# sdroh1027/DiffusionVID

Measured on AMD Instinct MI355X. Metric: frames/sec (1000x600) DiffusionVID-R101 x1, higher is better.
Workload: dtype f16

## Files before the change

### diffusionvid_amd/_lib.py

```python
import ctypes as C
import os

_HERE = os.path.dirname(os.path.abspath(__file__))
LIB_PATH = os.environ.get("DVID_LIB") or os.path.join(_HERE, "libdvid_hip.so")

c_void_p, c_int, c_float, c_int64 = C.c_void_p, C.c_int, C.c_float, C.c_int64
c_float_p = C.POINTER(C.c_float)


class DvidConfig(C.Structure):
    _fields_ = [
        ("hidden_dim", c_int), ("nheads", c_int), ("dim_feedforward", c_int), ("dim_dynamic", c_int),
        ("num_classes", c_int), ("num_cls", c_int), ("num_reg", c_int), ("num_heads", c_int),
        ("num_heads_cond", c_int), ("pooler_resolution", c_int), ("sampling_ratio", c_int),
        ("res_blocks", c_int * 4), ("pixel_mean", c_float * 3), ("pixel_std", c_float * 3),
        ("backbone_type", c_int), ("swin_embed_dim", c_int), ("swin_depths", c_int * 4), ("swin_heads", c_int * 4),
        ("swin_window", c_int),
    ]


SIGNATURES = {
    "dvid_last_error": (C.c_char_p, []),
    "dvid_version": (c_int, []),
    "dvid_model_create": (c_int, [C.POINTER(DvidConfig), C.POINTER(c_void_p)]),
# ... 40 lines not shown
    "dvid_noise_to_boxes": (c_int, [c_void_p, c_void_p, c_int, c_float, c_float, c_float, c_void_p]),
    "dvid_noise_to_boxes_sizes": (c_int, [c_void_p, c_void_p, c_int, c_int, c_float, c_void_p, c_void_p]),
    "dvid_ddim_renew_step_sizes": (c_int, [c_void_p] * 6 + [c_int] * 3 + [c_void_p] + [c_float] * 7 + [c_void_p]),
    "dvid_postproc_topk_nms_sizes": (c_int, [c_void_p, c_void_p, c_int, c_int, c_int, c_int, c_void_p, c_float, c_int,
                                             c_void_p, c_void_p, c_void_p, c_void_p, c_void_p, c_void_p]),
    "dvid_nms_frames_tiled_sizes": (c_int, [c_void_p] * 3 + [c_int, c_int, c_void_p, c_float, c_int, c_int] + [c_void_p] * 6),
    "dvid_ddim_renew_step": (c_int, [c_void_p] * 6 + [c_int] * 3 + [c_float] * 9 + [c_void_p]),
    "dvid_postproc_topk_nms": (c_int, [c_void_p, c_void_p, c_int, c_int, c_int, c_int, c_float, c_float, c_float, c_int,
                                       c_void_p, c_void_p, c_void_p, c_void_p, c_void_p, c_void_p]),
    "dvid_postproc_scratch_bytes": (c_int64, [c_int, c_int, c_int]),
    "dvid_topk_candidates_stream": (c_int, [c_void_p, c_void_p, c_int, c_int, c_int, c_int, c_void_p, c_void_p, c_void_p, c_void_p]),
    "dvid_nms_frames_tiled": (c_int, [c_void_p] * 3 + [c_int, c_int, c_float, c_float, c_float, c_int, c_int] + [c_void_p] * 6),
    "dvid_nms_tiled_scratch_bytes": (c_int64, [c_int, c_int]),
    "dvid_seq_nms_video": (c_int, [c_void_p] * 4 + [c_int] * 3 + [c_void_p] * 4 + [c_int64, c_void_p]),
    "dvid_seq_nms_scratch_bytes": (c_int64, [c_void_p, c_void_p, c_int, c_int]),
    "dvid_vid_eval_match": (c_int, [c_void_p, c_void_p, c_int, c_int] + [c_void_p] * 4 + [c_int, c_int] + [c_void_p] * 3 + [c_int, c_float, c_int] +
                            [c_void_p] * 7),
    "dvid_coco_eval_match": (c_int, [c_void_p, c_void_p, c_int, c_int] + [c_void_p] * 8 + [c_int] + [c_void_p] * 5),
    "dvid_lvis_eval_match": (c_int, [c_void_p, c_void_p, c_int, c_int] + [c_void_p] * 14 + [c_int] + [c_void_p] * 5),
    "dvid_eval_accumulate": (c_int, [c_void_p] * 6 + [c_int] * 5 + [c_void_p, c_int, c_void_p, c_int] + [c_void_p] * 3 + [c_int64, c_void_p]),
    "dvid_eval_accumulate_scratch_bytes": (c_int64, [c_int, c_int, c_int]),
    "dvid_cdist":(c_int, [c_void_p, c_int, c_int, c_void_p, c_void_p]),
    "dvid_fps_greedy": (c_int, [c_void_p, c_int, c_int, c_int, c_void_p, c_void_p]),
    "dvid_gather_rows": (c_int, [c_void_p, c_void_p, c_void_p, c_int, c_int, c_void_p]),
    "dvid_cdist_groups": (c_int, [c_void_p, c_int, c_int, c_int, c_void_p, c_void_p]),
    "dvid_fps_greedy_groups": (c_int, [c_void_p, c_int, c_int, c_int, c_int, c_void_p, c_void_p]),
    "dvid_gather_rows_groups": (c_int, [c_void_p, c_void_p, c_void_p, c_int, c_int, c_int, c_int, c_void_p]),
    "dvid_update_memory_groups": (c_int, [c_void_p, c_int, c_int, c_int, c_int, c_void_p, c_void_p, c_void_p, c_void_p]),
    "dvid_conv2d_nhwc_f16": (c_int, [c_void_p, c_void_p, c_void_p, c_void_p, c_void_p] + [c_int] * 13 + [c_void_p]),
    "dvid_bottleneck64_tail_f16": (c_int, [c_void_p] * 10 + [c_int] + [c_void_p] * 2 + [c_int] * 3 + [c_void_p]),
    "dvid_bottleneck128_tail_f16": (c_int, [c_void_p] * 10 + [c_int] * 3 + [c_void_p]),
    "dvid_mha_f16": (c_int, [c_void_p] * 5 + [c_int] * 7 + [c_int64] * 3 + [c_void_p]),
    "dvid_dynconv": (c_int, [c_void_p] * 7 + [c_int, c_void_p]),
    "dvid_add_layernorm": (c_int, [c_void_p] * 5 + [c_int, c_int, c_int, c_void_p]),
    "dvid_swin_pack_relbias": (c_int, [c_void_p, c_int, c_void_p]),
    "dvid_swin_window_attn_f16": (c_int, [c_void_p] * 4 + [c_int] * 6 + [c_void_p]),
    "dvid_swin_pack_relbias_ws": (c_int, [c_void_p, c_int, c_int, c_void_p]),
    "dvid_swin_window_attn_f16_ws": (c_int, [c_void_p] * 4 + [c_int] * 7 + [c_void_p]),
    "dvid_patch_merge_ln": (c_int, [c_void_p] * 5 + [c_int] * 4 + [c_void_p]),
    "dvid_nhwc_from_nchw": (c_int, [c_void_p, c_void_p, c_int, c_int, c_int, c_int, c_void_p]),
    "dvid_nchw_from_nhwc": (c_int, [c_void_p, c_void_p, c_int, c_int, c_int, c_int, c_void_p]),
    "dvid_f32_to_f16": (c_int, [c_void_p, c_void_p, c_int64, c_void_p]),
    "dvid_resize_u8_to_f32": (c_int, [c_void_p, c_int, c_int, c_void_p, c_void_p, c_int, c_int, c_int, c_int, c_void_p, c_void_p, c_int,
                                      c_void_p, c_void_p, c_int, c_void_p]),
    "dvid_resize_views_u8": (c_int, [c_void_p, c_int, c_void_p, c_void_p, c_void_p, c_int64, c_void_p, c_int64, c_void_p, c_int64, c_void_p, c_int, c_int,
                                     c_int, c_void_p]),
    "dvid_bbox_aug_merge": (c_int, [c_void_p] * 5 + [c_int] * 3 + [c_void_p] * 5),
    "dvid_overlay_detections": (c_int, [c_void_p] * 3 + [c_int, c_void_p, c_void_p, c_int, c_void_p, c_void_p, c_int, c_void_p, c_int, c_int,
                                        c_float, c_int, c_int, c_void_p, c_int64, c_void_p]),
    "dvid_overlay_scratch_bytes": (c_int64, [c_int, c_int]),
    "dvid_overlay_tile": (c_int, [C.POINTER(c_int), C.POINTER(c_int)]),
    "dvid_jpeg_parse": (c_int, [c_void_p, c_int64, c_void_p, c_void_p, c_int]),
    "dvid_jpeg_entropy_decode": (c_int, [c_void_p, c_int64, c_void_p, c_int64, c_void_p, c_void_p, c_int]),
    "dvid_jpeg_reconstruct_u8": (c_int, [c_void_p, c_int64, c_void_p, c_int64, c_void_p, c_void_p, c_int, c_void_p, c_int64, c_void_p, c_int64,
                                         c_void_p]),
    "dvid_igemm_num_configs": (c_int, []),
    "dvid_igemm_set_config": (c_int, [c_int]),
    "dvid_igemm_set_tuning": (c_int, [c_int]),
    "dvid_igemm_tuning_passes": (C.c_longlong, []),
    "dvid_igemm_set_conv3x3": (c_int, [c_int]),
    "dvid_igemm_set_wstat": (c_int, [c_int]),
    "dvid_igemm_set_bottleneck_fusion": (c_int, [c_int]),
    "dvid_set_stem_pool": (c_int, [c_int]),
    "dvid_set_option": (c_int, [C.c_char_p, c_int]),
    "dvid_get_option": (c_int, [C.c_char_p, C.POINTER(c_int)]),
    "dvid_reset_options": (c_int, []),
# ... 57 lines not shown
```

### diffusionvid_amd/csrc/dynconv.hip

```cpp
#include "common.h"
#include "f32_split.h"
#include "igemm_epilogue.h"
#include "kernels.h"
#include "options.h"
#include "roi_taps.h"

namespace {

constexpr int NP = 49;
constexpr int D = 256;
constexpr int DD = 64;
constexpr int A_PITCH = D + 8;
constexpr int H_PITCH = DD + 8;

__device__ __forceinline__ float groups4_sum(float v) {
    v += __shfl_xor(v, 16, 64);
    v += __shfl_xor(v, 32, 64);
    return v;
}

template <bool FUSED_ROI>
__global__ __launch_bounds__(256, 3) void dynconv_kernel(const half_t* __restrict__ roi, const half_t* __restrict__ params,
                                                       const float* __restrict__ g1, const float* __restrict__ b1,
                                                       const float* __restrict__ g2, const float* __restrict__ b2,
                                                       half_t* __restrict__ out, RoiLevels lv, const float* __restrict__ boxes,
                                                       int boxes_per_img, int nbox) {
    extern __shared__ __attribute__((aligned(16))) char smem[];
    half_t* As = reinterpret_cast<half_t*>(smem);
    half_t* Hs = As + 64 * A_PITCH;
    float* red = reinterpret_cast<float*>(Hs + 64 * H_PITCH);

    const int box = FUSED_ROI ? igemm_xcd_remap((int)blockIdx.x, nbox) : (int)blockIdx.x;
    const int tid = threadIdx.x, lane = tid & 63, wave = tid >> 6;
    const int l15 = lane & 15, l4 = lane >> 4;
    const half_t* p1t = params + (long)box * (2 * D * DD);
    const half_t* p2t = p1t + D * DD;
    const half8 zero8 = {0, 0, 0, 0, 0, 0, 0, 0};
    half8 bf[8];
    half8 b2f[4][2];

    if (FUSED_ROI) {
#pragma unroll
        for (int ks = 0; ks < 8; ++ks)
            bf[ks] = *reinterpret_cast<const half8*>(p1t + (wave * 16 + l15) * D + ks * 32 + l4 * 8);
#pragma unroll
        for (int nt = 0; nt < 4; ++nt)
#pragma unroll
            for (int ks = 0; ks < 2; ++ks)
                b2f[nt][ks] = *reinterpret_cast<const half8*>(p2t + (wave * 64 + nt * 16 + l15) * DD + ks * 32 + l4 * 8);
        float macc[8];
        roi_taps::gather_box(lv, boxes, boxes_per_img, box, tid >> 5, tid & 31, macc,
                             [&](int p, half8 o) { *reinterpret_cast<half8*>(As + p * A_PITCH + (tid & 31) * 8) = o; });
        for (int i = tid; i < (64 - NP) * 32; i += 256) *reinterpret_cast<half8*>(As + (NP + (i >> 5)) * A_PITCH + (i & 31) * 8) = zero8;
    } else {
        const half_t* roi_b = roi + (long)box * NP * D;
        for (int i = tid; i < 64 * 32; i += 256) {
            const int r = i >> 5, cv = i & 31;
            const half8 v = *reinterpret_cast<const half8*>(roi_b + (long)(r < NP ? r : 0) * D + cv * 8);
            *reinterpret_cast<half8*>(As + r * A_PITCH + cv * 8) = (r < NP) ? v : zero8;
        }
#pragma unroll
        for (int ks = 0; ks < 8; ++ks)
            bf[ks] = *reinterpret_cast<const half8*>(p1t + (wave * 16 + l15) * D + ks * 32 + l4 * 8);
    }
    __syncthreads();

    float4v acc1[4];
#pragma unroll
    for (int mt = 0; mt < 4; ++mt) acc1[mt] = (float4v){0.f, 0.f, 0.f, 0.f};
#pragma unroll
    for (int ks = 0; ks < 8; ++ks) {
#pragma unroll
        for (int mt = 0; mt < 4; ++mt) {
            const half8 af = *reinterpret_cast<const half8*>(As + (mt * 16 + l15) * A_PITCH + ks * 32 + l4 * 8);
            acc1[mt] = __builtin_amdgcn_mfma_f32_16x16x32_f16(bf[ks], af, acc1[mt], 0, 0, 0);
        }
    }
    if (!FUSED_ROI) {
#pragma unroll
        for (int nt = 0; nt < 4; ++nt)
#pragma unroll
            for (int ks = 0; ks < 2; ++ks)
                b2f[nt][ks] = *reinterpret_cast<const half8*>(p2t + (wave * 64 + nt * 16 + l15) * DD + ks * 32 + l4 * 8);
    }
// ... 90 lines not shown
    for (int nt = 0; nt < 4; ++nt) {
        const int col = wave * 64 + nt * 16 + l4 * 4;
        const float4v gg = *reinterpret_cast<const float4v*>(g2 + col), bb = *reinterpret_cast<const float4v*>(b2 + col);
#pragma unroll
        for (int mt = 0; mt < 4; ++mt) {
            half4 y;
#pragma unroll
            for (int r = 0; r < 4; ++r) y[r] = (half_t)fmaxf((acc2[mt][nt][r] - mean[mt]) * rstd[mt] * gg[r] + bb[r], 0.f);
            *reinterpret_cast<half4*>(As + (mt * 16 + l15) * A_PITCH + col) = y;
        }
    }
    __syncthreads();
    half_t* out_b = out + (long)box * NP * D;
    for (int i = tid; i < NP * 32; i += 256) {
        const int r = i >> 5, cv = i & 31;
        *reinterpret_cast<half8*>(out_b + (long)r * D + cv * 8) = *reinterpret_cast<const half8*>(As + r * A_PITCH + cv * 8);
    }
}

constexpr int kSmem = 64 * A_PITCH * 2 + 64 * H_PITCH * 2 + 64 * 4 * 4;

}

int dvid_dynconv_launch(const half_t* roi, const half_t* params, const float* g1, const float* b1, const float* g2,
                        const float* b2, half_t* out, int rows, hipStream_t s) {
    if (rows == 0) return DVID_OK;
    hipLaunchKernelGGL(dynconv_kernel<false>, dim3(rows), dim3(256), kSmem, s, roi, params, g1, b1, g2, b2, out, RoiLevels{}, nullptr, 1, rows);
    LAUNCH_CHECK();
    return DVID_OK;
}

int dvid_dynconv_roi_launch(const RoiLevels& lv, int channels, const float* boxes, int n_img, int boxes_per_img, const half_t* params,
                            const float* g1, const float* b1, const float* g2, const float* b2, half_t* out, hipStream_t s) {
    if (channels != 256) return DVID_ERR_UNSUPPORTED;
    const int rows = n_img * boxes_per_img;
    if (rows == 0) return DVID_OK;
    hipLaunchKernelGGL(dynconv_kernel<true>, dim3(rows), dim3(256), kSmem, s, nullptr, params, g1, b1, g2, b2, out, lv, boxes, boxes_per_img, rows);
    LAUNCH_CHECK();
    return DVID_OK;
}

namespace {

constexpr int DC_P1 = 68, DC_P2 = 260;
__global__ __launch_bounds__(256) __attribute__((amdgpu_waves_per_eu(2, 2))) void f32_dynconv_kernel(const float* __restrict__ roi, const float* __restrict__ params,
                                                           const float* __restrict__ g1, const float* __restrict__ b1,
                                                           const float* __restrict__ g2, const float* __restrict__ b2, float* __restrict__ out,
                                                           int nbox) {
#pragma clang fp contract(off)
    __shared__ float F1[64 * DC_P1];
    __shared__ float F2[49 * DC_P2];
    const int box = igemm_xcd_remap((int)blockIdx.x, nbox);
    const int tid = threadIdx.x, lane = tid & 63, wave = tid >> 6;
    const int fr = lane & 31, fk = (lane >> 5) * 4;
    const float* x = roi + (long)box * 49 * 256;
    const float* p1 = params + (long)box * 32768;
    const float* p2 = p1 + 64 * 256;

    float4v w2[2][8];
#pragma unroll
    for (int nb = 0; nb < 2; ++nb)
#pragma unroll
        for (int j = 0; j < 8; ++j) w2[nb][j] = *reinterpret_cast<const float4v*>(p2 + (long)((wave * 2 + nb) * 32 + fr) * 64 + j * 8 + fk);

    {
        const int mb = wave >> 1, nb = wave & 1;
        const int prow = mb * 32 + fr;
// ... 281 lines not shown
```

### diffusionvid_amd/csrc/model.hip

```cpp
#include <stdarg.h>

#include "runtime.h"

DvidOptions g_opt;

thread_local char g_err[512] = "";
void set_err(const char* fmt, ...) {
    va_list ap;
    va_start(ap, fmt);
    vsnprintf(g_err, sizeof(g_err), fmt, ap);
    va_end(ap);
}

int conv_run(const ConvW& w, const half_t* in, int n, int h, int wd, void* out, hipStream_t s, const ConvOpts& o) {
    IgemmParams p;
    memset(&p, 0, sizeof(p));
    p.in = in;
    p.w = w.w;
    p.bias = w.bias;
    p.res = o.res;
    p.out = out;
    p.H = h;
    p.W = wd;
    p.Cin = w.cin;
// ... 45 lines not shown
    p.wscale = w.wscale32;
    p.res = o.res;
    p.out = out;
    p.H = h;
    p.W = wd;
    p.Cin = w.cin32;
    p.KH = w.kh;
    p.KW = w.kw;
    p.stride = w.stride;
    p.pad = w.pad;
    p.Ho = (h + 2 * w.pad - w.kh) / w.stride + 1;
    p.Wo = (wd + 2 * w.pad - w.kw) / w.stride + 1;
    p.Cout = w.cout;
    p.M = n * p.Ho * p.Wo;
    p.K = w.kh * w.kw * w.cin32;
    p.Kpad = w.kpad32;
    p.ldc = o.ldc ? o.ldc : w.cout;
    p.relu = o.relu;
    p.res_mode = o.res_mode;
    if (o.ho_out) *o.ho_out = p.Ho;
    if (o.wo_out) *o.wo_out = p.Wo;
    const double alg_k = (double)w.kh * w.kw * (w.cin_real ? w.cin_real : w.cin32);
    const double in_px = (double)p.M * (w.kh * w.kw > 1 ? w.stride * w.stride : 1);
    const double bytes = 4.0 * (in_px * p.Cin + (double)p.Cout * p.Kpad + (double)p.M * p.Cout * (o.res_mode == 1 ? 2.0 : o.res_mode == 2 ? 1.25 : 1.0));
    return prof_other("igemm_f32", p.M, p.Cout, p.Kpad, 2.0 * p.M * (double)p.Cout * alg_k, bytes, s, [&] { return dvid_f32_igemm_launch(p, s); },
                      true);
}
int linear_run32(const ConvW& w, const float* in, int rows, float* out, int relu, hipStream_t s, int ldc) {
    return conv_run32(w, in, rows, 1, 1, out, s, {.relu = relu, .ldc = ldc});
}

extern "C" {
const char* dvid_last_error(void) { return g_err; }
int dvid_version(void) { return 11; }

int dvid_model_create(const dvid_config* cfg, dvid_model** out) {
    g_err[0] = 0;
    if (!cfg || !out) FAIL(DVID_ERR_ARG, "null argument");
    if (cfg->hidden_dim != 256 || cfg->nheads != 8 || cfg->dim_dynamic != 64 || cfg->pooler_resolution != 7 ||
        cfg->sampling_ratio != 2)
        FAIL(DVID_ERR_UNSUPPORTED,
             "kernels are specialised for HIDDEN_DIM 256, NHEADS 8, DIM_DYNAMIC 64, POOLER_RESOLUTION 7, SAMPLING_RATIO 2");
    if (cfg->dim_feedforward % 64) FAIL(DVID_ERR_UNSUPPORTED, "DIM_FEEDFORWARD must be a multiple of 64");
    if (cfg->num_classes < 1 || cfg->num_classes > DVID_MAX_CLASSES)
        FAIL(DVID_ERR_UNSUPPORTED, "NUM_CLASSES %d: 1 <= NUM_CLASSES <= DVID_MAX_CLASSES = %d", cfg->num_classes, DVID_MAX_CLASSES);
    int dev_count = 0;
    if (hipGetDeviceCount(&dev_count) != hipSuccess || dev_count == 0) FAIL(DVID_ERR_HIP, "no HIP device available");
    dvid_model* m = new dvid_model();
    m->cfg = *cfg;
    if (const char* e = getenv("DVID_CHAINS")) m->nchain = atoi(e) < 1 ? 1 : (atoi(e) > 4 ? 4 : atoi(e));
    *out = m;
    return DVID_OK;
}

int dvid_model_destroy(dvid_model* m) {
    if (!m) return DVID_OK;
    for (void* p : m->owned) (void)hipFree(p);
    delete m;
    return DVID_OK;
}

int dvid_model_set_precision(dvid_model* m, int precision) {
    g_err[0] = 0;
    if (!m || (precision != 0 && precision != 1)) FAIL(DVID_ERR_ARG, "precision must be 0 (float16) or 1 (float32)");
    if (m->finalized) FAIL(DVID_ERR_STATE, "dvid_model_set_precision must precede dvid_model_finalize (the weights are packed for one precision)");
    m->precision = precision;
    return DVID_OK;
// ... 163 lines not shown
```

### diffusionvid_amd/csrc/ops_abi.hip

```cpp
#include "runtime.h"

extern "C" {
int dvid_roialign_v2_multilevel(const void* p3, const void* p4, const void* p5, int n_frames, int height, int width, int channels,
                                const float* boxes, int boxes_per_frame, void* roi_out, float* mean_out, void* stream) {
    const void* levels[3] = {p3, p4, p5};
    return dvid_roialign_v2_levels(levels, 3, n_frames, height, width, channels, boxes, boxes_per_frame, roi_out, mean_out, stream);
}

int dvid_roialign_v2_levels(const void* const* levels, int n_levels, int n_frames, int height, int width, int channels, const float* boxes,
                            int boxes_per_frame, void* roi_out, float* mean_out, void* stream) {
    g_err[0] = 0;
    if (!pyramid_ok(levels, n_levels)) FAIL(DVID_ERR_ARG, "the pyramid is 3 maps (p3..p5) or 4 (p2..p5), none of them null (got n_levels %d)", n_levels);
    if (height % 32 || width % 32) FAIL(DVID_ERR_ARG, "height/width must be multiples of 32");
    TRY(dvid_roialign_launch(roi_levels<half_t>(levels, n_levels, height, width, 0, channels), channels, boxes, n_frames, boxes_per_frame,
                             reinterpret_cast<half_t*>(roi_out), mean_out, reinterpret_cast<hipStream_t>(stream)));
    return DVID_OK;
}

int dvid_roialign_v2_multilevel_f32(const float* p3, const float* p4, const float* p5, int n_frames, int height, int width, int channels,
                                    const float* boxes, int boxes_per_frame, float* roi_out, float* mean_out, void* stream) {
    const float* levels[3] = {p3, p4, p5};
    return dvid_roialign_v2_levels_f32(levels, 3, n_frames, height, width, channels, boxes, boxes_per_frame, roi_out, mean_out, stream);
}

// ... 483 lines not shown
    const int rc = bneck_tail(reinterpret_cast<const half_t*>(t1), reinterpret_cast<const half_t*>(w2), b2, reinterpret_cast<const half_t*>(w3),
                              b3, reinterpret_cast<const half_t*>(residual), reinterpret_cast<const half_t*>(w_shortcut), b_shortcut,
                              reinterpret_cast<const half_t*>(w1_next), b1_next, next_channels, reinterpret_cast<half_t*>(out),
                              reinterpret_cast<half_t*>(t1_next), n, h, wd, reinterpret_cast<hipStream_t>(stream));
    if (rc != DVID_OK) FAIL(rc, "bottleneck tail: bad argument (n %d, %d x %d, next conv1 with %d channels)", n, h, wd, next_channels);
    return DVID_OK;
}

int dvid_bottleneck128_tail_f16(const void* t1, const void* w2, const float* b2, const void* w3, const float* b3, const void* residual,
                                const void* w1_next, const float* b1_next, void* out, void* t1_next, int n, int h, int wd, void* stream) {
    g_err[0] = 0;
    const int rc = bneck128_tail(reinterpret_cast<const half_t*>(t1), reinterpret_cast<const half_t*>(w2), b2, reinterpret_cast<const half_t*>(w3),
                                 b3, reinterpret_cast<const half_t*>(residual), reinterpret_cast<const half_t*>(w1_next), b1_next,
                                 reinterpret_cast<half_t*>(out), reinterpret_cast<half_t*>(t1_next), n, h, wd,
                                 reinterpret_cast<hipStream_t>(stream));
    if (rc != DVID_OK) FAIL(rc, "bottleneck tail (128): bad argument (n %d, %d x %d)", n, h, wd);
    return DVID_OK;
}

int dvid_mha_f16(const void* q, const void* k, const void* v, void* out, void* vt_scratch, int batch, int lq, int lk, int nheads,
                 int q_ld, int kv_ld, int out_ld, int64_t q_bs, int64_t kv_bs, int64_t out_bs, void* stream) {
    g_err[0] = 0;
    TRY(dvid_mha_mfma_launch(reinterpret_cast<const half_t*>(q), reinterpret_cast<const half_t*>(k), reinterpret_cast<const half_t*>(v),
                             reinterpret_cast<half_t*>(out), reinterpret_cast<half_t*>(vt_scratch), batch, lq, lk, nheads, q_ld, kv_ld,
                             out_ld, q_bs, kv_bs, out_bs, reinterpret_cast<hipStream_t>(stream)));
    return DVID_OK;
}

int dvid_dynconv(const void* roi, const void* params, const float* g1, const float* b1, const float* g2, const float* b2, void* out,
                 int rows, void* stream) {
    g_err[0] = 0;
    TRY(dvid_dynconv_launch(reinterpret_cast<const half_t*>(roi), reinterpret_cast<const half_t*>(params), g1, b1, g2, b2,
                            reinterpret_cast<half_t*>(out), rows, reinterpret_cast<hipStream_t>(stream)));
    return DVID_OK;
}

int dvid_add_layernorm(const float* x, const float* r, const float* g, const float* b, float* y, int rows, int d, int relu,
                       void* stream) {
    g_err[0] = 0;
    TRY(dvid_add_layernorm_launch(x, r, g, b, y, nullptr, rows, d, relu, reinterpret_cast<hipStream_t>(stream)));
    return DVID_OK;
}

int dvid_swin_window_attn_f16(const void* qkv, const void* qkv_bias16, const float* relbias, void* out, int batch, int H, int W, int C,
                              int nheads, int shift, void* stream) {
    g_err[0] = 0;
    if (!qkv || !qkv_bias16 || !relbias || !out) FAIL(DVID_ERR_ARG, "swin window attention: null pointer");
    if (batch <= 0 || H <= 0 || W <= 0 || nheads <= 0 || shift < 0 || shift >= 7)
        FAIL(DVID_ERR_ARG, "swin window attention: bad sizes (batch %d, %d x %d tokens, %d heads, shift %d)", batch, H, W, nheads, shift);
    const int rc = dvid_swin_window_attn_launch(reinterpret_cast<const half_t*>(qkv), reinterpret_cast<const half_t*>(qkv_bias16), relbias,
                                                reinterpret_cast<half_t*>(out), batch, H, W, C, nheads, shift, reinterpret_cast<hipStream_t>(stream));
    if (rc != DVID_OK) FAIL(rc, "swin window attention: C %d with %d heads on %d x %d x %d tokens is not supported", C, nheads, batch, H, W);
    return DVID_OK;
}

int dvid_swin_window_attn_f16_ws(const void* qkv, const void* qkv_bias16, const float* relbias, void* out, int batch, int H, int W, int C,
                                 int nheads, int shift, int window, void* stream) {
    if (window == 7) return dvid_swin_window_attn_f16(qkv, qkv_bias16, relbias, out, batch, H, W, C, nheads, shift, stream);
    g_err[0] = 0;
    if (window != 12) FAIL(DVID_ERR_UNSUPPORTED, "swin window attention: window size %d (7 and 12 are built)", window);
    if (!qkv || !qkv_bias16 || !relbias || !out) FAIL(DVID_ERR_ARG, "swin window attention: null pointer");
    if (batch <= 0 || H <= 0 || W <= 0 || nheads <= 0 || shift < 0 || shift >= window)
        FAIL(DVID_ERR_ARG, "swin window attention: bad sizes (batch %d, %d x %d tokens, %d heads, shift %d, window %d)", batch, H, W, nheads, shift, window);
    const int rc = dvid_swin_window12_attn_launch(reinterpret_cast<const half_t*>(qkv), reinterpret_cast<const half_t*>(qkv_bias16), relbias,
                                                  reinterpret_cast<half_t*>(out), batch, H, W, C, nheads, shift, reinterpret_cast<hipStream_t>(stream));
    if (rc != DVID_OK) FAIL(rc, "swin window attention (window 12): C %d with %d heads on %d x %d x %d tokens is not supported", C, nheads, batch, H, W);
// ... 173 lines not shown
```

### diffusionvid_amd/csrc/roi_taps.h

```cpp
#pragma once

#include "common.h"
#include "kernels.h"

namespace roi_taps {

constexpr int P = 7;
constexpr int G = 2;
constexpr int CV = 32;

typedef unsigned int uint4v __attribute__((ext_vector_type(4)));
__device__ __forceinline__ float mix_fma_lo(unsigned int h2, float w, float acc) {
    float d;
    asm("v_fma_mix_f32 %0, %1, %2, %3 op_sel_hi:[1,0,0]" : "=v"(d) : "v"(h2), "v"(w), "v"(acc));
    return d;
}
__device__ __forceinline__ float mix_fma_hi(unsigned int h2, float w, float acc) {
    float d;
    asm("v_fma_mix_f32 %0, %1, %2, %3 op_sel:[1,0,0] op_sel_hi:[1,0,0]" : "=v"(d) : "v"(h2), "v"(w), "v"(acc));
    return d;
}
__device__ __forceinline__ void tap_fma8(float (&acc)[8], half8 v, float w) {
    const uint4v u = __builtin_bit_cast(uint4v, v);
#pragma unroll
    for (int q = 0; q < 4; ++q) {
        acc[2 * q] = mix_fma_lo(u[q], w, acc[2 * q]);
        acc[2 * q + 1] = mix_fma_hi(u[q], w, acc[2 * q + 1]);
    }
}

struct Tap {
    int lo, hi;
    float wl, wh;
    bool ok;
};

__device__ __forceinline__ Tap axis_tap(float y, int limit) {
    Tap t;
    t.ok = !(y < -1.0f || y > (float)limit);
    if (y <= 0.f) y = 0.f;
    int lo = (int)y;
    int hi;
    if (lo >= limit - 1) {
        hi = lo = limit - 1;
        y = (float)lo;
    } else {
        hi = lo + 1;
    }
    const float l = y - (float)lo;
    t.lo = lo;
    t.hi = hi;
    t.wl = 1.f - l;
    t.wh = l;
    return t;
}

__device__ __forceinline__ int box_level(float bx1, float by1, float bx2, float by2, int min_level, bool& valid) {
    const float area = (bx2 - bx1) * (by2 - by1);
    valid = area >= 0.f;
    float lvf = floorf(4.f + log2f(sqrtf(area) / 224.f + 1e-8f));
    lvf = fminf(fmaxf(lvf, (float)min_level), 5.f);
    return valid ? (int)lvf - min_level : 0;
}

template <typename Sink>
__device__ __forceinline__ void gather_box(const RoiLevels& lv, const float* __restrict__ boxes, int boxes_per_img, int box, int grp, int ln,
                                           float (&macc)[8], Sink&& sink) {
    const int img = box / boxes_per_img;
    const float bx1 = boxes[box * 4 + 0], by1 = boxes[box * 4 + 1], bx2 = boxes[box * 4 + 2], by2 = boxes[box * 4 + 3];
    bool valid_box;
    const int level = box_level(bx1, by1, bx2, by2, lv.min_level, valid_box);

    const half_t* feat = lv.feat[level];
    const int H = lv.h[level], W = lv.w[level];
    const float sc = lv.scale[level];
    feat += (long)img * H * W * (CV * 8);

    const float x1 = bx1 * sc - 0.5f, y1 = by1 * sc - 0.5f;
    const float x2 = bx2 * sc - 0.5f, y2 = by2 * sc - 0.5f;
    const float bin_w = (x2 - x1) / P, bin_h = (y2 - y1) / P;

#pragma unroll
    for (int e = 0; e < 8; ++e) macc[e] = 0.f;

    for (int p = grp; p < P * P; p += 8) {
        const int ph = p / P, pw = p - ph * P;
        float acc[8];
#pragma unroll
        for (int e = 0; e < 8; ++e) acc[e] = 0.f;
        if (valid_box) {
#pragma unroll
            for (int iy = 0; iy < G; ++iy) {
                const float y = y1 + ph * bin_h + (iy + 0.5f) * bin_h / G;
                const Tap ty = axis_tap(y, H);
#pragma unroll
                for (int ix = 0; ix < G; ++ix) {
                    const float x = x1 + pw * bin_w + (ix + 0.5f) * bin_w / G;
                    const Tap tx = axis_tap(x, W);
                    if (!(ty.ok && tx.ok)) continue;
                    const half8 v1 = *reinterpret_cast<const half8*>(feat + ((long)ty.lo * W + tx.lo) * (CV * 8) + ln * 8);
                    const half8 v2 = *reinterpret_cast<const half8*>(feat + ((long)ty.lo * W + tx.hi) * (CV * 8) + ln * 8);
                    const half8 v3 = *reinterpret_cast<const half8*>(feat + ((long)ty.hi * W + tx.lo) * (CV * 8) + ln * 8);
                    const half8 v4 = *reinterpret_cast<const half8*>(feat + ((long)ty.hi * W + tx.hi) * (CV * 8) + ln * 8);
                    const float w1 = ty.wl * tx.wl, w2 = ty.wl * tx.wh, w3 = ty.wh * tx.wl, w4 = ty.wh * tx.wh;
                    tap_fma8(acc, v1, w1);
                    tap_fma8(acc, v2, w2);
                    tap_fma8(acc, v3, w3);
                    tap_fma8(acc, v4, w4);
                }
            }
        }
        half8 o;
#pragma unroll
        for (int e = 0; e < 8; ++e) {
            acc[e] *= 1.f / (G * G);
            macc[e] += acc[e];
            o[e] = (half_t)acc[e];
        }
        sink(p, o);
    }
}

}
```

### diffusionvid_amd/csrc/roialign.hip

```cpp
#include <stdlib.h>

#include "common.h"
#include "igemm_epilogue.h"
#include "kernels.h"
#include "roi_taps.h"

namespace {

using namespace roi_taps;

__global__ __launch_bounds__(256) void roialign_kernel(RoiLevels lv, const float* __restrict__ boxes, int boxes_per_img,
                                                        half_t* __restrict__ roi_out, float* __restrict__ mean_out, int nbox,
                                                        int xcd_major) {
    __shared__ float red[8][256];
    const int box = xcd_major ? igemm_xcd_remap((int)blockIdx.x, nbox) : (int)blockIdx.x;
    const int tid = threadIdx.x;
    const int grp = tid >> 5, ln = tid & 31;
    float macc[8];
    gather_box(lv, boxes, boxes_per_img, box, grp, ln, macc,
               [&](int p, half8 o) { *reinterpret_cast<half8*>(roi_out + ((long)box * (P * P) + p) * (CV * 8) + ln * 8) = o; });
    if (mean_out) {
#pragma unroll
        for (int e = 0; e < 8; ++e) red[grp][ln * 8 + e] = macc[e];
        __syncthreads();
        float s = 0.f;
#pragma unroll
        for (int g = 0; g < 8; ++g) s += red[g][tid];
        mean_out[(long)box * 256 + tid] = s / (P * P);
    }
}

__global__ __launch_bounds__(256) void f32_roialign_kernel(RoiLevels32 lv, const float* __restrict__ boxes, int boxes_per_img,
                                                            float* __restrict__ roi_out, float* __restrict__ mean_out, int nbox) {
#pragma clang fp contract(off)
    __shared__ float red[8][256];
    const int box = igemm_xcd_remap((int)blockIdx.x, nbox);
    const int img = box / boxes_per_img;
    const int tid = threadIdx.x;
    const int grp = tid >> 5, ln = tid & 31;
    const float bx1 = boxes[box * 4 + 0], by1 = boxes[box * 4 + 1], bx2 = boxes[box * 4 + 2], by2 = boxes[box * 4 + 3];
    bool valid_box;
    const int level = box_level(bx1, by1, bx2, by2, lv.min_level, valid_box);
    const int H = lv.h[level], W = lv.w[level];
    const float sc = lv.scale[level];
    const float* feat = lv.feat[level] + (long)img * H * W * 256;
    const float x1 = bx1 * sc - 0.5f, y1 = by1 * sc - 0.5f;
    const float x2 = bx2 * sc - 0.5f, y2 = by2 * sc - 0.5f;
    const float bin_w = (x2 - x1) / P, bin_h = (y2 - y1) / P;
    float macc[8];
#pragma unroll
    for (int e = 0; e < 8; ++e) macc[e] = 0.f;
    for (int pb = grp; pb < P * P; pb += 8) {
// ... 20 lines not shown
#pragma unroll
                        for (int e = 0; e < 4; ++e) {
                            acc[e] += w4[q] * a[e];
                            acc[4 + e] += w4[q] * b[e];
                        }
                    }
                }
            }
        }
#pragma unroll
        for (int e = 0; e < 8; ++e) {
            acc[e] *= 1.f / (G * G);
            macc[e] += acc[e];
        }
        float* o = roi_out + ((long)box * (P * P) + pb) * 256 + ln * 8;
        *reinterpret_cast<float4v*>(o) = (float4v){acc[0], acc[1], acc[2], acc[3]};
        *reinterpret_cast<float4v*>(o + 4) = (float4v){acc[4], acc[5], acc[6], acc[7]};
    }
    if (mean_out) {
#pragma unroll
        for (int e = 0; e < 8; ++e) red[grp][ln * 8 + e] = macc[e];
        __syncthreads();
        float s = 0.f;
#pragma unroll
        for (int g = 0; g < 8; ++g) s += red[g][tid];
        mean_out[(long)box * 256 + tid] = s / (P * P);
    }
}

}

int dvid_roialign_launch(const RoiLevels& lv, int channels, const float* boxes, int n_img, int boxes_per_img, half_t* roi_out,
                         float* mean_out, hipStream_t s) {
    if (channels != 256) return DVID_ERR_UNSUPPORTED;
    const int nbox = n_img * boxes_per_img;
    if (nbox == 0) return DVID_OK;
    hipLaunchKernelGGL(roialign_kernel, dim3(nbox), dim3(256), 0, s, lv, boxes, boxes_per_img, roi_out, mean_out, nbox, 1);
    LAUNCH_CHECK();
    return DVID_OK;
}

int dvid_f32_roialign_launch(const RoiLevels32& lv, int channels, const float* boxes, int n_img, int boxes_per_img, float* roi_out,
                             float* mean_out, hipStream_t s) {
    if (channels != 256) return DVID_ERR_UNSUPPORTED;
    const int nbox = n_img * boxes_per_img;
    if (nbox == 0) return DVID_OK;
    hipLaunchKernelGGL(f32_roialign_kernel, dim3(nbox), dim3(256), 0, s, lv, boxes, boxes_per_img, roi_out, mean_out, nbox);
    LAUNCH_CHECK();
    return DVID_OK;
}
```

### diffusionvid_amd/ops.py

```python
import ctypes as C

import torch

from . import _lib
from ._lib import call, ptr, stream_ptr


def _cuda(t, dtype=None):
    if not t.is_cuda:
        raise _lib.DvidError("libdvid_hip ops need tensors on the GPU (no CPU fallback)")
    if dtype is not None and t.dtype != dtype:
        raise TypeError(f"expected {dtype}, got {t.dtype}")
    return t.contiguous()


def nhwc_from_nchw(x):
    x = _cuda(x, torch.float32)
    n, c, h, w = x.shape
    out = torch.empty((n, h, w, c), dtype=torch.float16, device=x.device)
    call("dvid_nhwc_from_nchw", ptr(x), ptr(out), n, h, w, c, stream_ptr())
    return out


def nchw_from_nhwc(x):
# ... 147 lines not shown
    feats = [_cuda(f, torch.float16) for f in feats_nhwc]
    levels, nl = _pyramid(feats, height, width, "roialign")
    boxes = _cuda(boxes, torch.float32)
    n, M = boxes.shape[:2]
    c = feats[0].shape[-1]
    roi = torch.empty((n * M, 49, c), dtype=torch.float16, device=boxes.device)
    mean = torch.empty((n * M, c), dtype=torch.float32, device=boxes.device) if want_mean else None
    call("dvid_roialign_v2_levels", levels, nl, n, height, width, c, ptr(boxes), M, ptr(roi), ptr(mean), stream_ptr())
    return (roi, mean) if want_mean else roi


def mha_f16(q, k, v, nheads):
    def h(t):
        t = _cuda(t)
        if t.dtype == torch.float16:
            return t
        o = torch.empty(t.shape, dtype=torch.float16, device=t.device)
        call("dvid_f32_to_f16", ptr(t), ptr(o), t.numel(), stream_ptr())
        return o
    q, k, v = h(q), h(k), h(v)
    B, lq, d = q.shape
    lk = k.shape[1]
    out = torch.empty_like(q)
    vt = torch.empty((B * nheads * 32 * ((lk + 31) // 32 * 32 + 32),), dtype=torch.float16, device=q.device)
    call("dvid_mha_f16", ptr(q), ptr(k), ptr(v), ptr(out), ptr(vt), B, lq, lk, nheads, d, d, d, lq * d, lk * d, lq * d,
         stream_ptr())
    return out


def dynconv(roi16, params16, g1, b1, g2, b2):
    roi16, params16 = _cuda(roi16, torch.float16), _cuda(params16, torch.float16)
    out = torch.empty_like(roi16)
    call("dvid_dynconv", ptr(roi16), ptr(params16), ptr(g1), ptr(b1), ptr(g2), ptr(b2), ptr(out), roi16.shape[0], stream_ptr())
    return out


def add_layernorm(x, r, g, b, relu=False):
    x = _cuda(x, torch.float32)
    y = torch.empty_like(x)
    call("dvid_add_layernorm", ptr(x), ptr(r), ptr(g), ptr(b), ptr(y), x.shape[0], x.shape[1], int(relu), stream_ptr())
    return y


def _swin_relbias_pitch(window):
    return (window * window + 31) // 32 * 32


def swin_pack_relbias(table, window=7):
    table = table.detach().cpu().contiguous()
    if table.dtype != torch.float32 or table.dim() != 2 or table.shape[0] != (2 * window - 1) ** 2:
        raise TypeError(f"expected a float32 [{(2 * window - 1) ** 2}, heads] table, got {table.dtype} {tuple(table.shape)}")
    out = torch.empty((table.shape[1], window * window, _swin_relbias_pitch(window)), dtype=torch.float32)
    if window == 7:
        call("dvid_swin_pack_relbias", ptr(table), table.shape[1], ptr(out))
    else:
        call("dvid_swin_pack_relbias_ws", ptr(table), table.shape[1], window, ptr(out))
    return out


def _swin_window_attn(name, dtype, qkv, qkv_bias, relbias, B, H, W, nheads, shift, out, window):
    qkv, qkv_bias, relbias = _cuda(qkv, dtype), _cuda(qkv_bias, dtype), _cuda(relbias, torch.float32)
    C = qkv.shape[1] // 3
    assert tuple(qkv.shape) == (B * H * W, 3 * C) and qkv_bias.numel() == 3 * C
    assert tuple(relbias.shape) == (nheads, window * window, _swin_relbias_pitch(window))
    if out is None:
        out = torch.empty((B * H * W, C), dtype=dtype, device=qkv.device)
# ... 829 lines not shown
```

### include/dvid_hip.h

```cpp
#ifndef DVID_HIP_H
#define DVID_HIP_H

#include <stdint.h>

#ifdef __cplusplus
extern "C" {
#endif

#define DVID_OK 0
#define DVID_ERR_ARG 1
#define DVID_ERR_HIP 2
#define DVID_ERR_UNSUPPORTED 3
#define DVID_ERR_STATE 4

#define DVID_MAX_CLASSES 1280

typedef struct dvid_model dvid_model;

typedef struct dvid_config {
    int hidden_dim;
    int nheads;
    int dim_feedforward;
    int dim_dynamic;
    int num_classes;
// ... 136 lines not shown
int dvid_lvis_eval_match(const float* dets, const int* counts, int n_images, int cap, const double* gt_boxes, const double* gt_areas,
                         const unsigned char* gt_ignore, const int* gt_labels, const int* gt_starts, const int* gt_starts_host,
                         const int* neg_starts, const int* neg_labels, const int* neg_starts_host, const int* nex_starts, const int* nex_labels,
                         const int* nex_starts_host, const double* iou_thrs, const double* area_ranges, int num_classes, signed char* match,
                         signed char* ignore, int* rank, int* npig, void* stream);
#define DVID_EVAL_ACCUMULATE_RECALLS 101
#define DVID_EVAL_ACCUMULATE_MAX_LIMITS 3
#define DVID_EVAL_ACCUMULATE_MAX_SCRATCH_BYTES (1ll << 30)
int dvid_eval_accumulate(const float* dets, const int* counts, const int* rank, const signed char* match, const signed char* ignore,
                         const int* npig, int n_images, int cap, int num_classes, int n_areas, int n_thresholds, const int* max_dets,
                         int max_dets_count, const double* rec_thrs, int n_rec_thrs, double* precision, double* recall, void* scratch,
                         long long scratch_bytes, void* stream);
long long dvid_eval_accumulate_scratch_bytes(int n_images, int cap, int max_dets_count);
int dvid_cdist(const float* x, int n, int d, float* dist, void* stream);
int dvid_fps_greedy(const float* dist, int n, int m, int bs_emul, int* idx, void* stream);
int dvid_gather_rows(const float* x, const int* idx, float* y, int m, int d, void* stream);
#define DVID_UPDATE_MEMORY_MAX_SCRATCH_BYTES (1ll << 30)
int dvid_cdist_groups(const float* x, int groups, int n, int d, float* dist, void* stream);
int dvid_fps_greedy_groups(const float* dist, int groups, int n, int m, int bs_emul, int* idx, void* stream);
int dvid_gather_rows_groups(const float* x, const int* idx, float* y, int groups, int n, int m, int d, void* stream);
int dvid_update_memory_groups(const float* merged, int groups, int n, int d, int m, float* dist_scratch, int* idx, float* out, void* stream);
int dvid_conv2d_nhwc_f16(const void* in, const void* w, const float* bias, const void* residual, void* out, int n, int h,
                         int wd, int cin, int cout, int kh, int kw, int stride, int pad, int kpad, int relu, int out_f32,
                         int residual_mode, void* stream);
int dvid_bottleneck64_tail_f16(const void* t1, const void* w2, const float* b2, const void* w3, const float* b3, const void* residual,
                               const void* w_shortcut, const float* b_shortcut, const void* w1_next, const float* b1_next, int next_channels,
                               void* out, void* t1_next, int n, int h, int wd, void* stream);
int dvid_bottleneck128_tail_f16(const void* t1, const void* w2, const float* b2, const void* w3, const float* b3, const void* residual,
                                const void* w1_next, const float* b1_next, void* out, void* t1_next, int n, int h, int wd, void* stream);
int dvid_mha_f16(const void* q, const void* k, const void* v, void* out, void* vt_scratch, int batch, int lq, int lk, int nheads,
                 int q_ld, int kv_ld, int out_ld, int64_t q_bs, int64_t kv_bs, int64_t out_bs, void* stream);
int dvid_dynconv(const void* roi, const void* params, const float* g1, const float* b1, const float* g2, const float* b2,
                 void* out, int rows, void* stream);
int dvid_add_layernorm(const float* x, const float* r, const float* g, const float* b, float* y, int rows, int d, int relu,
                       void* stream);
int dvid_swin_pack_relbias(const float* table, int nheads, float* out);
int dvid_swin_window_attn_f16(const void* qkv, const void* qkv_bias16, const float* relbias, void* out, int batch, int H, int W, int C,
                              int nheads, int shift, void* stream);
int dvid_swin_pack_relbias_ws(const float* table, int nheads, int window, float* out);
int dvid_swin_window_attn_f16_ws(const void* qkv, const void* qkv_bias16, const float* relbias, void* out, int batch, int H, int W, int C,
                                 int nheads, int shift, int window, void* stream);
int dvid_patch_merge_ln(const float* x, const float* g, const float* b, void* y16, float* y32, int B, int H, int W, int C, void* stream);
int dvid_nhwc_from_nchw(const float* in, void* out_f16, int n, int h, int w, int c, void* stream);
int dvid_nchw_from_nhwc(const void* in_f16, float* out, int n, int h, int w, int c, void* stream);
int dvid_f32_to_f16(const float* x, void* y, int64_t n, void* stream);

int dvid_resize_u8_to_f32(const void* src_hwc, int h, int w, void* tmp, float* out_chw, int oh, int ow, int ph, int pw,
                          const int* xbounds, const int* xk, int xksize, const int* ybounds, const int* yk, int yksize, void* stream);

int dvid_resize_views_u8(const void* const* srcs, int n, const long long* plan, const long long* plan_host, const int* bounds,
                         int64_t n_bound_rows, const int* weights, int64_t n_weights, void* tmp, int64_t tmp_bytes, float* out, int ph, int pw,
                         int flip, void* stream);
#define DVID_BBOX_AUG_MAX_VIEWS 64
int dvid_bbox_aug_merge(const float* boxes, const float* scores, const int* labels, const int* counts, const float* table, int n, int views,
                        int cap, float* cand_boxes, float* cand_scores, int* cand_labels, int* live, void* stream);

#define DVID_OVERLAY_MAX_DRAWN 256
#define DVID_OVERLAY_NAME_MAX 24
int dvid_overlay_detections(void* const* frames, const int* sizes, const int* sizes_host, int n, const float* dets, const int* counts, int cap,
                            const float* ratios, const unsigned char* names, int num_classes, const unsigned char* atlas, int gh, int gw,
                            float threshold, int thickness, int text_scale, void* scratch, int64_t scratch_bytes, void* stream);
int64_t dvid_overlay_scratch_bytes(int n, int cap);
int dvid_overlay_tile(int* tile_w, int* tile_h);

typedef struct dvid_jpeg_info {
    int32_t width, height, ncomp;
// ... 41 lines not shown
```

Before: 2378.

## Batch RoIAlign bilinear loads across samples and expose fused RoI dynconv entry point

Templates gather_box on a sample count. The standalone RoIAlign kernel now issues the loads for all four bilinear samples before accumulating, and uses 32-bit unsigned offsets, which is guarded by a new check on map size. The fused dynconv path keeps one sample at a time to limit register pressure. The change also pins down FMA contraction so results are deterministic, adds a public ABI and Python wrapper for the fused RoIAlign+DynamicConv kernel, and bumps the library version. Batching the loads costs more registers in exchange for more loads in flight.

```diff
diff --git a/diffusionvid_amd/_lib.py b/diffusionvid_amd/_lib.py
--- a/diffusionvid_amd/_lib.py
+++ b/diffusionvid_amd/_lib.py
@@ -96,6 +96,7 @@
     "dvid_bottleneck128_tail_f16": (c_int, [c_void_p] * 10 + [c_int] * 3 + [c_void_p]),
     "dvid_mha_f16": (c_int, [c_void_p] * 5 + [c_int] * 7 + [c_int64] * 3 + [c_void_p]),
     "dvid_dynconv": (c_int, [c_void_p] * 7 + [c_int, c_void_p]),
+    "dvid_dynconv_roi": (c_int, [c_void_p, c_int, c_int, c_int, c_int, c_void_p, c_int] + [c_void_p] * 7),
     "dvid_add_layernorm": (c_int, [c_void_p] * 5 + [c_int, c_int, c_int, c_void_p]),
     "dvid_swin_pack_relbias": (c_int, [c_void_p, c_int, c_void_p]),
     "dvid_swin_window_attn_f16": (c_int, [c_void_p] * 4 + [c_int] * 6 + [c_void_p]),
diff --git a/diffusionvid_amd/csrc/dynconv.hip b/diffusionvid_amd/csrc/dynconv.hip
--- a/diffusionvid_amd/csrc/dynconv.hip
+++ b/diffusionvid_amd/csrc/dynconv.hip
@@ -49,7 +49,7 @@
             for (int ks = 0; ks < 2; ++ks)
                 b2f[nt][ks] = *reinterpret_cast<const half8*>(p2t + (wave * 64 + nt * 16 + l15) * DD + ks * 32 + l4 * 8);
         float macc[8];
-        roi_taps::gather_box(lv, boxes, boxes_per_img, box, tid >> 5, tid & 31, macc,
+        roi_taps::gather_box<1>(lv, boxes, boxes_per_img, box, tid >> 5, tid & 31, macc,
                              [&](int p, half8 o) { *reinterpret_cast<half8*>(As + p * A_PITCH + (tid & 31) * 8) = o; });
         for (int i = tid; i < (64 - NP) * 32; i += 256) *reinterpret_cast<half8*>(As + (NP + (i >> 5)) * A_PITCH + (i & 31) * 8) = zero8;
     } else {
@@ -206,7 +206,7 @@
 
 int dvid_dynconv_roi_launch(const RoiLevels& lv, int channels, const float* boxes, int n_img, int boxes_per_img, const half_t* params,
                             const float* g1, const float* b1, const float* g2, const float* b2, half_t* out, hipStream_t s) {
-    if (channels != 256) return DVID_ERR_UNSUPPORTED;
+    if (channels != 256 || !roi_taps::maps_addressable(lv)) return DVID_ERR_UNSUPPORTED;
     const int rows = n_img * boxes_per_img;
     if (rows == 0) return DVID_OK;
     hipLaunchKernelGGL(dynconv_kernel<true>, dim3(rows), dim3(256), kSmem, s, nullptr, params, g1, b1, g2, b2, out, lv, boxes, boxes_per_img, rows);
diff --git a/diffusionvid_amd/csrc/model.hip b/diffusionvid_amd/csrc/model.hip
--- a/diffusionvid_amd/csrc/model.hip
+++ b/diffusionvid_amd/csrc/model.hip
@@ -101,7 +101,7 @@
 
 extern "C" {
 const char* dvid_last_error(void) { return g_err; }
-int dvid_version(void) { return 11; }
+int dvid_version(void) { return 12; }
 
 int dvid_model_create(const dvid_config* cfg, dvid_model** out) {
     g_err[0] = 0;
diff --git a/diffusionvid_amd/csrc/ops_abi.hip b/diffusionvid_amd/csrc/ops_abi.hip
--- a/diffusionvid_amd/csrc/ops_abi.hip
+++ b/diffusionvid_amd/csrc/ops_abi.hip
@@ -539,6 +539,19 @@
     g_err[0] = 0;
     TRY(dvid_dynconv_launch(reinterpret_cast<const half_t*>(roi), reinterpret_cast<const half_t*>(params), g1, b1, g2, b2,
                             reinterpret_cast<half_t*>(out), rows, reinterpret_cast<hipStream_t>(stream)));
+    return DVID_OK;
+}
+
+int dvid_dynconv_roi(const void* const* levels, int n_levels, int n_frames, int height, int width, const float* boxes, int boxes_per_frame,
+                     const void* params, const float* g1, const float* b1, const float* g2, const float* b2, void* out, void* stream) {
+    g_err[0] = 0;
+    if (!pyramid_ok(levels, n_levels)) FAIL(DVID_ERR_ARG, "the pyramid is 3 maps (p3..p5) or 4 (p2..p5), none of them null (got n_levels %d)", n_levels);
+    if (height % 32 || width % 32) FAIL(DVID_ERR_ARG, "height/width must be multiples of 32");
+    if (n_frames < 0 || boxes_per_frame < 0 || !boxes || !params || !g1 || !b1 || !g2 || !b2 || !out)
+        FAIL(DVID_ERR_ARG, "fused RoIAlign + DynamicConv: null pointer or negative count (%d frames x %d boxes)", n_frames, boxes_per_frame);
+    TRY(dvid_dynconv_roi_launch(roi_levels<half_t>(levels, n_levels, height, width, 0, 256), 256, boxes, n_frames, boxes_per_frame,
+                                reinterpret_cast<const half_t*>(params), g1, b1, g2, b2, reinterpret_cast<half_t*>(out),
+                                reinterpret_cast<hipStream_t>(stream)));
     return DVID_OK;
 }
 
diff --git a/diffusionvid_amd/csrc/roi_taps.h b/diffusionvid_amd/csrc/roi_taps.h
--- a/diffusionvid_amd/csrc/roi_taps.h
+++ b/diffusionvid_amd/csrc/roi_taps.h
@@ -1,33 +1,20 @@
 #pragma once
 
+#if defined(__HIPCC__)
 #include "common.h"
 #include "kernels.h"
+#define ROI_TAPS_HD __host__ __device__ __forceinline__
+#else
+#include <math.h>
+#define ROI_TAPS_HD inline
+#endif
 
 namespace roi_taps {
 
 constexpr int P = 7;
 constexpr int G = 2;
 constexpr int CV = 32;
-
-typedef unsigned int uint4v __attribute__((ext_vector_type(4)));
-__device__ __forceinline__ float mix_fma_lo(unsigned int h2, float w, float acc) {
-    float d;
-    asm("v_fma_mix_f32 %0, %1, %2, %3 op_sel_hi:[1,0,0]" : "=v"(d) : "v"(h2), "v"(w), "v"(acc));
-    return d;
-}
-__device__ __forceinline__ float mix_fma_hi(unsigned int h2, float w, float acc) {
-    float d;
-    asm("v_fma_mix_f32 %0, %1, %2, %3 op_sel:[1,0,0] op_sel_hi:[1,0,0]" : "=v"(d) : "v"(h2), "v"(w), "v"(acc));
-    return d;
-}
-__device__ __forceinline__ void tap_fma8(float (&acc)[8], half8 v, float w) {
-    const uint4v u = __builtin_bit_cast(uint4v, v);
-#pragma unroll
-    for (int q = 0; q < 4; ++q) {
-        acc[2 * q] = mix_fma_lo(u[q], w, acc[2 * q]);
-        acc[2 * q + 1] = mix_fma_hi(u[q], w, acc[2 * q + 1]);
-    }
-}
+constexpr long kMaxMapPixels = 1L << 22;
 
 struct Tap {
     int lo, hi;
@@ -35,7 +22,30 @@
     bool ok;
 };
 
-__device__ __forceinline__ Tap axis_tap(float y, int limit) {
+ROI_TAPS_HD Tap axis_tap(float y, int limit) {
+    Tap t;
+    t.ok = !(y < -1.0f || y > (float)limit);
+    if (y <= 0.f) y = 0.f;
+    const float top = (float)limit;
+    const float yc = y > 0.f ? (y < top ? y : top) : 0.f;
+    int lo = (int)yc;
+    if (lo < 0) lo = 0;
+    int hi;
+    if (lo >= limit - 1) {
+        hi = lo = limit - 1;
+        y = (float)lo;
+    } else {
+        hi = lo + 1;
+    }
+    const float l = y - (float)lo;
+    t.lo = lo;
+    t.hi = hi;
+    t.wl = 1.f - l;
+    t.wh = l;
+    return t;
+}
+
+ROI_TAPS_HD Tap axis_tap_counted(float y, int limit) {
     Tap t;
     t.ok = !(y < -1.0f || y > (float)limit);
     if (y <= 0.f) y = 0.f;
@@ -55,7 +65,7 @@
     return t;
 }
 
-__device__ __forceinline__ int box_level(float bx1, float by1, float bx2, float by2, int min_level, bool& valid) {
+ROI_TAPS_HD int box_level(float bx1, float by1, float bx2, float by2, int min_level, bool& valid) {
     const float area = (bx2 - bx1) * (by2 - by1);
     valid = area >= 0.f;
     float lvf = floorf(4.f + log2f(sqrtf(area) / 224.f + 1e-8f));
@@ -63,9 +73,48 @@
     return valid ? (int)lvf - min_level : 0;
 }
 
-template <typename Sink>
+}
+
+#if defined(__HIPCC__)
+namespace roi_taps {
+
+inline bool maps_addressable(const RoiLevels& lv) {
+    for (int l = 0; l < lv.n_levels; ++l)
+        if ((long)lv.h[l] * lv.w[l] > kMaxMapPixels) return false;
+    return true;
+}
+
+typedef unsigned int uint4v __attribute__((ext_vector_type(4)));
+__device__ __forceinline__ float mix_fma_lo(unsigned int h2, float w, float acc) {
+    float d;
+    asm("v_fma_mix_f32 %0, %1, %2, %3 op_sel_hi:[1,0,0]" : "=v"(d) : "v"(h2), "v"(w), "v"(acc));
+    return d;
+}
+__device__ __forceinline__ float mix_fma_hi(unsigned int h2, float w, float acc) {
+    float d;
+    asm("v_fma_mix_f32 %0, %1, %2, %3 op_sel:[1,0,0] op_sel_hi:[1,0,0]" : "=v"(d) : "v"(h2), "v"(w), "v"(acc));
+    return d;
+}
+__device__ __forceinline__ void tap_fma8(float (&acc)[8], half8 v, float w) {
+    const uint4v u = __builtin_bit_cast(uint4v, v);
+#pragma unroll
+    for (int q = 0; q < 4; ++q) {
+        acc[2 * q] = mix_fma_lo(u[q], w, acc[2 * q]);
+        acc[2 * q + 1] = mix_fma_hi(u[q], w, acc[2 * q + 1]);
+    }
+}
+__device__ __forceinline__ void sample_fma(float (&acc)[8], const half8 (&v)[4], const Tap& ty, const Tap& tx) {
+#pragma clang fp contract(off)
+    tap_fma8(acc, v[0], ty.wl * tx.wl);
+    tap_fma8(acc, v[1], ty.wl * tx.wh);
+    tap_fma8(acc, v[2], ty.wh * tx.wl);
+    tap_fma8(acc, v[3], ty.wh * tx.wh);
+}
+
+template <int SAMPLES, typename Sink>
 __device__ __forceinline__ void gather_box(const RoiLevels& lv, const float* __restrict__ boxes, int boxes_per_img, int box, int grp, int ln,
                                            float (&macc)[8], Sink&& sink) {
+#pragma clang fp contract(off)
     const int img = box / boxes_per_img;
     const float bx1 = boxes[box * 4 + 0], by1 = boxes[box * 4 + 1], bx2 = boxes[box * 4 + 2], by2 = boxes[box * 4 + 3];
     bool valid_box;
@@ -76,8 +125,8 @@
     const float sc = lv.scale[level];
     feat += (long)img * H * W * (CV * 8);
 
-    const float x1 = bx1 * sc - 0.5f, y1 = by1 * sc - 0.5f;
-    const float x2 = bx2 * sc - 0.5f, y2 = by2 * sc - 0.5f;
+    const float x1 = __builtin_fmaf(bx1, sc, -0.5f), y1 = __builtin_fmaf(by1, sc, -0.5f);
+    const float x2 = __builtin_fmaf(bx2, sc, -0.5f), y2 = __builtin_fmaf(by2, sc, -0.5f);
     const float bin_w = (x2 - x1) / P, bin_h = (y2 - y1) / P;
 
 #pragma unroll
@@ -88,37 +137,66 @@
         float acc[8];
 #pragma unroll
         for (int e = 0; e < 8; ++e) acc[e] = 0.f;
-        if (valid_box) {
+        if (valid_box && SAMPLES == 1) {
 #pragma unroll
             for (int iy = 0; iy < G; ++iy) {
-                const float y = y1 + ph * bin_h + (iy + 0.5f) * bin_h / G;
-                const Tap ty = axis_tap(y, H);
+                const float y = __builtin_fmaf((float)ph, bin_h, y1) + (iy + 0.5f) * bin_h / G;
+                const Tap ty = axis_tap_counted(y, H);
 #pragma unroll
                 for (int ix = 0; ix < G; ++ix) {
-                    const float x = x1 + pw * bin_w + (ix + 0.5f) * bin_w / G;
-                    const Tap tx = axis_tap(x, W);
+                    const float x = __builtin_fmaf((float)pw, bin_w, x1) + (ix + 0.5f) * bin_w / G;
+                    const Tap tx = axis_tap_counted(x, W);
                     if (!(ty.ok && tx.ok)) continue;
-                    const half8 v1 = *reinterpret_cast<const half8*>(feat + ((long)ty.lo * W + tx.lo) * (CV * 8) + ln * 8);
-                    const half8 v2 = *reinterpret_cast<const half8*>(feat + ((long)ty.lo * W + tx.hi) * (CV * 8) + ln * 8);
-                    const half8 v3 = *reinterpret_cast<const half8*>(feat + ((long)ty.hi * W + tx.lo) * (CV * 8) + ln * 8);
-                    const half8 v4 = *reinterpret_cast<const half8*>(feat + ((long)ty.hi * W + tx.hi) * (CV * 8) + ln * 8);
-                    const float w1 = ty.wl * tx.wl, w2 = ty.wl * tx.wh, w3 = ty.wh * tx.wl, w4 = ty.wh * tx.wh;
-                    tap_fma8(acc, v1, w1);
-                    tap_fma8(acc, v2, w2);
-                    tap_fma8(acc, v3, w3);
-                    tap_fma8(acc, v4, w4);
+                    half8 v[4];
+                    v[0] = *reinterpret_cast<const half8*>(feat + ((long)ty.lo * W + tx.lo) * (CV * 8) + ln * 8);
+                    v[1] = *reinterpret_cast<const half8*>(feat + ((long)ty.lo * W + tx.hi) * (CV * 8) + ln * 8);
+                    v[2] = *reinterpret_cast<const half8*>(feat + ((long)ty.hi * W + tx.lo) * (CV * 8) + ln * 8);
+                    v[3] = *reinterpret_cast<const half8*>(feat + ((long)ty.hi * W + tx.hi) * (CV * 8) + ln * 8);
+                    sample_fma(acc, v, ty, tx);
+                }
+            }
+        } else if (valid_box) {
+            Tap ty[G], tx[G];
+#pragma unroll
+            for (int i = 0; i < G; ++i) {
+                ty[i] = axis_tap(__builtin_fmaf((float)ph, bin_h, y1) + (i + 0.5f) * bin_h / G, H);
+                tx[i] = axis_tap(__builtin_fmaf((float)pw, bin_w, x1) + (i + 0.5f) * bin_w / G, W);
+            }
+            auto load4 = [&](half8 (&v)[4], const Tap& y, const Tap& x) {
+                const unsigned row_lo = (unsigned)y.lo * (unsigned)W, row_hi = (unsigned)y.hi * (unsigned)W;
+                v[0] = *reinterpret_cast<const half8*>(feat + ((row_lo + x.lo) * (CV * 8) + ln * 8));
+                v[1] = *reinterpret_cast<const half8*>(feat + ((row_lo + x.hi) * (CV * 8) + ln * 8));
+                v[2] = *reinterpret_cast<const half8*>(feat + ((row_hi + x.lo) * (CV * 8) + ln * 8));
+                v[3] = *reinterpret_cast<const half8*>(feat + ((row_hi + x.hi) * (CV * 8) + ln * 8));
+            };
+#pragma unroll
+            for (int s0 = 0; s0 < G * G; s0 += SAMPLES) {
+                half8 v[SAMPLES][4];
+                bool inside = true;
+#pragma unroll
+                for (int s = 0; s < SAMPLES; ++s) {
+                    inside = inside && ty[(s0 + s) / G].ok && tx[(s0 + s) % G].ok;
+                    load4(v[s], ty[(s0 + s) / G], tx[(s0 + s) % G]);
+                }
+                if (inside) {
+#pragma unroll
+                    for (int s = 0; s < SAMPLES; ++s) sample_fma(acc, v[s], ty[(s0 + s) / G], tx[(s0 + s) % G]);
+                } else {
+#pragma unroll
+                    for (int s = 0; s < SAMPLES; ++s)
+                        if (ty[(s0 + s) / G].ok && tx[(s0 + s) % G].ok) sample_fma(acc, v[s], ty[(s0 + s) / G], tx[(s0 + s) % G]);
                 }
             }
         }
         half8 o;
 #pragma unroll
         for (int e = 0; e < 8; ++e) {
-            acc[e] *= 1.f / (G * G);
-            macc[e] += acc[e];
-            o[e] = (half_t)acc[e];
+            macc[e] = __builtin_fmaf(acc[e], 1.f / (G * G), macc[e]);
+            o[e] = (half_t)(acc[e] * (1.f / (G * G)));
         }
         sink(p, o);
     }
 }
 
 }
+#endif
diff --git a/diffusionvid_amd/csrc/roialign.hip b/diffusionvid_amd/csrc/roialign.hip
--- a/diffusionvid_amd/csrc/roialign.hip
+++ b/diffusionvid_amd/csrc/roialign.hip
@@ -17,7 +17,7 @@
     const int tid = threadIdx.x;
     const int grp = tid >> 5, ln = tid & 31;
     float macc[8];
-    gather_box(lv, boxes, boxes_per_img, box, grp, ln, macc,
+    gather_box<4>(lv, boxes, boxes_per_img, box, grp, ln, macc,
                [&](int p, half8 o) { *reinterpret_cast<half8*>(roi_out + ((long)box * (P * P) + p) * (CV * 8) + ln * 8) = o; });
     if (mean_out) {
 #pragma unroll
@@ -104,7 +104,7 @@
 
 int dvid_roialign_launch(const RoiLevels& lv, int channels, const float* boxes, int n_img, int boxes_per_img, half_t* roi_out,
                          float* mean_out, hipStream_t s) {
-    if (channels != 256) return DVID_ERR_UNSUPPORTED;
+    if (channels != 256 || !maps_addressable(lv)) return DVID_ERR_UNSUPPORTED;
     const int nbox = n_img * boxes_per_img;
     if (nbox == 0) return DVID_OK;
     hipLaunchKernelGGL(roialign_kernel, dim3(nbox), dim3(256), 0, s, lv, boxes, boxes_per_img, roi_out, mean_out, nbox, 1);
diff --git a/diffusionvid_amd/ops.py b/diffusionvid_amd/ops.py
--- a/diffusionvid_amd/ops.py
+++ b/diffusionvid_amd/ops.py
@@ -203,6 +203,20 @@
     roi16, params16 = _cuda(roi16, torch.float16), _cuda(params16, torch.float16)
     out = torch.empty_like(roi16)
     call("dvid_dynconv", ptr(roi16), ptr(params16), ptr(g1), ptr(b1), ptr(g2), ptr(b2), ptr(out), roi16.shape[0], stream_ptr())
+    return out
+
+
+def dynconv_roi(feats_nhwc, boxes, height, width, params16, g1, b1, g2, b2):
+    feats = [_cuda(f, torch.float16) for f in feats_nhwc]
+    levels, nl = _pyramid(feats, height, width, "dynconv_roi")
+    if feats[0].shape[-1] != 256:
+        raise _lib.DvidError(f"dynconv_roi: the maps must have 256 channels, got {feats[0].shape[-1]}")
+    boxes, params16 = _cuda(boxes, torch.float32), _cuda(params16, torch.float16)
+    n, M = boxes.shape[:2]
+    if params16.numel() != n * M * 32768:
+        raise _lib.DvidError(f"dynconv_roi: {n * M} boxes need {n * M} x 32768 parameters, got {params16.numel()}")
+    out = torch.empty((n * M, 49, 256), dtype=torch.float16, device=boxes.device)
+    call("dvid_dynconv_roi", levels, nl, n, height, width, ptr(boxes), M, ptr(params16), ptr(g1), ptr(b1), ptr(g2), ptr(b2), ptr(out), stream_ptr())
     return out
 
 
diff --git a/include/dvid_hip.h b/include/dvid_hip.h
--- a/include/dvid_hip.h
+++ b/include/dvid_hip.h
@@ -192,6 +192,8 @@
                  int q_ld, int kv_ld, int out_ld, int64_t q_bs, int64_t kv_bs, int64_t out_bs, void* stream);
 int dvid_dynconv(const void* roi, const void* params, const float* g1, const float* b1, const float* g2, const float* b2,
                  void* out, int rows, void* stream);
+int dvid_dynconv_roi(const void* const* levels, int n_levels, int n_frames, int height, int width, const float* boxes, int boxes_per_frame,
+                     const void* params, const float* g1, const float* b1, const float* g2, const float* b2, void* out, void* stream);
 int dvid_add_layernorm(const float* x, const float* r, const float* g, const float* b, float* y, int rows, int d, int relu,
                        void* stream);
 int dvid_swin_pack_relbias(const float* table, int nheads, float* out);
```

After: 2365. Within noise of the previous version (-0.5%).
